# MVME-HBUT/Faster-OreFSDet

Measured on AMD Instinct MI355X. Metric: images/sec at 640x640 25-shot (eval FPS: model(inputs) + device sync per image, bs=1 per GPU), higher is better.
Workload: dtype f32

## Files before the change

### faster-orefsdet_amd/csrc/ore_conv_internal.h

```cpp
#pragma once
#include "ore_common.h"

namespace oreconv {

struct Lvl { int orow0, irow0, H, W, Ho, Wo; };

struct ConvP {
    const float* in; int in_ld, in_coff;
    int B, Cin;
    int nlev; Lvl lv[4];
    const float* w;
    int Cout, Cout16, kh, kw, stride, pad, M, K;
    const float* scale; const float* shift; int ep_stride; int relu_cout;
    const float* in_mul; const float* in_add; int in_relu;
    const float* add; int add_ld, add_coff, add_H, add_W;
    float* out; int out_ld, out_coff;
    float* colsum;
    int splitk, steps_per_split, nchunks;
    float* ws; int* tile_cnt;
    int bf16;
    int xmap;
    int sb;
    const float* wino;
    size_t w_lstride;
// ... 1 lines not shown
};

__device__ __forceinline__ void tile_of_block(int xmap, int& bx, int& by) {
    bx = blockIdx.x; by = blockIdx.y;
    if (xmap == 0) return;
    const int gx = gridDim.x, gy = gridDim.y, T = gx * gy;
    const int lin = by * gx + bx, r = lin & 7, k = lin >> 3;
    const int q = T >> 3, rem = T & 7;
    const int t = r * q + min(r, rem) + k;
    if (xmap == 1) { bx = t / gy; by = t - bx * gy; }
    else { by = t / gx; bx = t - by * gx; }
}

__device__ __forceinline__ void decode_row(const ConvP& p, int m, int& lvl, int& b, int& oy, int& ox) {
    lvl = 0;
#pragma unroll
    for (int l = 1; l < 4; ++l)
        if (l < p.nlev && m >= p.lv[l].orow0) lvl = l;
    const Lvl& L = p.lv[lvl];
    const int r = m - L.orow0, hw = L.Ho * L.Wo;
    b = r / hw;
    const int q = r - b * hw;
    oy = q / L.Wo;
    ox = q - oy * L.Wo;
}

constexpr unsigned kOOB = 0x80000000u;
constexpr int kGdTab = 64;
constexpr int kKdTab = 512;
constexpr int kRfTab = 256;

#define ORE_IGEMM_BUILDS(X)                                                                                                         \
                                                                         \
    X(128, 16, 4, 1, 1, 0) X(128, 32, 4, 1, 1, 0) X(128, 48, 4, 1, 1, 0) X(128, 64, 4, 1, 1, 0)                                     \
    X(128, 80, 4, 1, 1, 0) X(128, 96, 4, 1, 1, 0) X(128, 112, 4, 1, 1, 0) X(128, 128, 2, 2, 1, 0)                                   \
    X(64, 16, 4, 1, 1, 1) X(64, 32, 4, 1, 1, 1) X(64, 48, 4, 1, 1, 1) X(64, 64, 4, 1, 1, 1)                                         \
    X(64, 80, 4, 1, 1, 1) X(64, 96, 4, 1, 1, 1) X(64, 112, 4, 1, 1, 1) X(64, 128, 2, 2, 1, 1)                                       \
                                                                            \
    X(64, 64, 2, 1, 2, 0) X(64, 32, 2, 1, 2, 0) X(64, 16, 2, 1, 2, 0) X(64, 48, 2, 1, 2, 0)                                         \
    X(32, 64, 1, 1, 4, 0) X(32, 48, 1, 1, 4, 0) X(32, 32, 1, 1, 4, 1) X(32, 16, 1, 1, 4, 0)                                         \
    X(16, 64, 1, 1, 4, 0) X(16, 48, 1, 1, 4, 0) X(16, 32, 1, 1, 4, 1) X(16, 16, 1, 1, 4, 1)                                         \
    X(64, 128, 2, 1, 2, 0) X(64, 96, 2, 1, 2, 0) X(64, 80, 2, 1, 2, 0) X(64, 112, 2, 1, 2, 0)                                       \
    X(32, 128, 1, 1, 4, 0) X(32, 96, 1, 1, 4, 0) X(32, 80, 1, 1, 4, 0) X(32, 112, 1, 1, 4, 0)                                       \
    X(32, 128, 2, 1, 2, 0) X(32, 64, 2, 1, 2, 1) X(32, 32, 2, 1, 2, 0)                                                              \
    X(128, 64, 2, 1, 2, 0) X(128, 128, 2, 1, 2, 0)
#define ORE_GD_BUILDS(X)                                                                                                            \
    X(64, 128, 2, 2, 4, 1) X(64, 64, 2, 2, 4, 1) X(32, 64, 1, 4, 4, 1)                                                              \
    X(64, 128, 2, 2, 4, 0) X(64, 64, 2, 2, 4, 0) X(64, 112, 4, 1, 4, 0) X(128, 64, 4, 1, 4, 0) X(128, 128, 2, 2, 4, 0)              \
    X(32, 128, 1, 4, 4, 0) X(128, 112, 4, 1, 4, 0) X(208, 64, 1, 4, 4, 0) X(224, 64, 1, 4, 4, 0) X(112, 64, 1, 4, 4, 0)             \
    X(96, 128, 2, 2, 4, 0) X(64, 128, 2, 2, 2, 0) X(128, 128, 2, 2, 2, 0) X(208, 64, 1, 4, 2, 0) X(128, 112, 4, 1, 2, 0)            \
    X(128, 128, 2, 4, 4, 0) X(112, 128, 1, 8, 4, 0) X(128, 112, 8, 1, 4, 0) X(64, 128, 2, 4, 4, 0) X(128, 64, 4, 2, 4, 0)           \
    X(64, 64, 2, 4, 4, 0) X(128, 128, 2, 4, 2, 0) X(112, 128, 1, 8, 2, 0) X(80, 64, 1, 4, 4, 0) X(80, 128, 1, 4, 4, 0)              \
    X(48, 64, 1, 4, 4, 0) X(32, 64, 1, 4, 4, 0)
#define ORE_KD_BUILDS(X)                                                                                                            \
    X(16, 16, 4, 4) X(16, 16, 4, 8) X(16, 16, 8, 4) X(16, 16, 16, 2) X(16, 32, 4, 4) X(16, 32, 8, 2) X(32, 32, 4, 4) X(32, 32, 8, 2)  \
    X(16, 48, 4, 4) X(16, 48, 8, 2) X(16, 64, 4, 2) X(16, 80, 4, 2) X(32, 64, 4, 2) X(32, 80, 4, 2) X(64, 64, 4, 2) X(32, 48, 4, 2)    \
    X(32, 16, 4, 4)
#define ORE_RF_BUILDS(X) \
    X(1, 4, 8) X(1, 4, 12) X(1, 4, 16) X(1, 8, 12) X(1, 8, 16) X(1, 8, 20) X(1, 16, 12) X(2, 4, 12) X(2, 4, 16) X(2, 8, 12)
#define ORE_GS_BUILDS(X) \
    X(64, 112, 4, 1) X(64, 128, 2, 2) X(64, 64, 2, 2) X(128, 64, 4, 1) X(128, 128, 2, 2) X(32, 128, 1, 4) X(128, 112, 4, 1) X(64, 80, 4, 1) X(32, 64, 2, 2)
#define ORE_KW_TILES(X) \
    X(16, 16) X(16, 32) X(16, 48) X(16, 64) X(16, 80) X(32, 16) X(32, 32) X(32, 48) X(32, 64) X(32, 80)
constexpr bool gs_fits(int bm, int bn, int ns) { return ((bm + bn) / 16 + 3) / 4 * (ns - 1) <= 63 && (size_t)ns * (bm + bn) * 64 <= 150 * 1024; }

struct ConvKnobs {
    int patch_mode = -1;
    int kw_mode = 1;
    int kw_force[4] = {};
    int gs_force[2] = {};
    int gs_ns = 3;
    int xmap_force = -1;
    int kw_nw_force = 0;
    int wino_mode = 1;
    int ws_sb_mode = 1;
    int ws_s2_mode = 1;
    int rf_mode = 1;
    int rf_force[3] = {};
    int kd_mode = 1;
    int kd_force[4] = {};
    int gd_mode = 1;
    int gd_force[3] = {};
    int gd_dbg = 0;
    int igemm[5] = {};
};
extern ConvKnobs g_knobs;

using ConvPlan = ore_conv_plan_t;
ConvPlan conv_plan(const ConvP& p, int req_splitk, size_t workspace_floats);
bool conv_wino_covers(int Cout, int Cin);
int wino_level_blocks(const ConvP& p, int gy, int* blk0);

int launch_ws(const ConvP& p, const ConvPlan& pl, hipStream_t st);
int launch_patch(const ConvP& p, const ConvPlan& pl, hipStream_t st);
int launch_igemm(const ConvP& p, const ConvPlan& pl, hipStream_t st);
int launch_wino(const ConvP& p, const ConvPlan& pl, hipStream_t st);
int launch_gd(const ConvP& p, const ConvPlan& pl, hipStream_t st);
int launch_kd(const ConvP& p, const ConvPlan& pl, hipStream_t st);
int launch_rf(const ConvP& p, const ConvPlan& pl, hipStream_t st);
int launch_gs(const ConvP& p, const ConvPlan& pl, hipStream_t st);
int launch_kw(const ConvP& p, const ConvPlan& pl, hipStream_t st);
int conv_gd_splitk(const float* in, int in_ld, const float* w, int M, int K, int Cout16, float* parts, int S, hipStream_t st);

int launch_wgrad_reduce(const float* slab, int S, int Cout, int taps, int Cin, float beta, float* dw_oihw, long long stride, float* db,
                        float beta_b, hipStream_t st);

}
```

### faster-orefsdet_amd/csrc/ore_conv_plan.cpp

```cpp
#include "ore_common.h"
#include "ore_conv_internal.h"

namespace oreconv {

ConvKnobs g_knobs;

namespace {

const ConvKnobs& K = g_knobs;

ConvPlan make_plan(int launcher, int bm, int bn, int b0, int b1, int b2, int b3, int gx, int gy, int xmap = 0, int splitk = 1, int sps = 0) {
    ConvPlan pl{};
    pl.launcher = launcher; pl.error = ORE_OK;
    pl.bm = bm; pl.bn = bn;
    pl.build[0] = b0; pl.build[1] = b1; pl.build[2] = b2; pl.build[3] = b3;
    pl.splitk = splitk; pl.steps_per_split = sps; pl.xmap = xmap;
    pl.gx = gx; pl.gy = gy;
    return pl;
}

ConvPlan none() { return ConvPlan{}; }

ConvPlan fail(int code) {
    ConvPlan pl{};
// ... 430 lines not shown
}

}

bool conv_wino_covers(int Cout, int Cin) {
    if (Cout <= 0 || Cout % 16 != 0) return false;
    if (Cin == 64) return Cout % 64 == 0;
    if (Cin == 128) return Cout % 32 == 0;
    return Cin == 80 || Cin == 96 || Cin == 112;
}

int wino_level_blocks(const ConvP& c, int gy, int* blk0) {
    int nb[4];
    for (int l = 0; l < c.nlev; ++l) nb[l] = c.B * ceil_div(c.lv[l].W, 16) * ceil_div(c.lv[l].H, 4);
    const int G = 256 / gy > c.nlev ? 256 / gy : c.nlev;
    int R = 1;
    for (;; ++R) {
        int need = 0;
        for (int l = 0; l < c.nlev; ++l) need += ceil_div(nb[l], R);
        if (need <= G) break;
    }
    int gx = 0;
    for (int l = 0; l < c.nlev; ++l) { if (blk0) blk0[l] = gx; gx += ceil_div(nb[l], R); }
    if (blk0) blk0[c.nlev] = gx;
    return gx;
}

ConvPlan conv_plan(const ConvP& p, int req_splitk, size_t workspace_floats) {
    ConvPlan pl;
    if (p.w_lstride) {
        if ((pl = plan_ws_sb(p)).launcher) return pl;
        ore_set_error("ore_conv2d_levels_fwd: the weight-stationary bf16 kernel does not cover this per-level launch (64 / 128 channels, Cout %% 64 == 0)");
        return fail(ORE_EINVAL);
    }
    if (p.wino_lstride) {
        if ((pl = plan_wino(p)).launcher) return pl;
        ore_set_error("ore_conv2d_levels_fwd: the Winograd kernel does not cover this per-level launch (alignment / mode)");
        return fail(ORE_EINVAL);
    }
    if (p.sb & 1) {
        if ((pl = plan_ws_sb(p)).launcher || (pl = plan_ws_s2(p)).launcher) return pl;
        pl = plan_dma(p, workspace_floats);
        if (pl.launcher || pl.error) return pl;
        ore_set_error("ore_conv2d_fwd: no bf16-storage kernel for this layer (input affine?)");
        return fail(ORE_EINVAL);
    }
    if (K.igemm[0] == 0 && req_splitk <= 1) {
        if ((pl = plan_wino(p)).launcher) return pl;
        if (K.kw_mode && ((pl = plan_gd(p)).launcher || pl.error)) return pl;
        const bool kw_first = K.kw_mode == 2 || (K.kw_mode == 1 && p.nlev > 1);
        if (!kw_first && (pl = plan_patch(p)).launcher) return pl;
        if (K.kw_mode) {
            pl = plan_dma(p, workspace_floats);
            if (pl.launcher || pl.error) return pl;
            if (kw_first && K.kw_mode != 2 && (pl = plan_patch(p)).launcher) return pl;
        }
    }
    return plan_igemm(p, req_splitk, workspace_floats);
}

}

using namespace oreconv;

extern "C" int ore_conv_set_plan_override(int32_t BM, int32_t BN, int32_t WGM, int32_t WGN, int32_t WGK) {
    ConvKnobs& k = g_knobs;
    switch (BM) {
    case -1: k.patch_mode = BN; k.igemm[0] = 0; break;
    case -2: k.kw_mode = BN; k.igemm[0] = 0; break;
    case -3: k.kw_force[0] = BN; k.kw_force[1] = WGM; k.kw_force[2] = WGN; k.kw_force[3] = WGK; break;
    case -4: k.gs_force[0] = BN; k.gs_force[1] = WGM; if (WGN > 0) k.gs_ns = WGN; break;
    case -5: k.xmap_force = BN; break;
    case -6: k.kw_nw_force = BN; break;
    case -7: k.wino_mode = BN; break;
    case -8: k.ws_sb_mode = BN; break;
    case -9: k.ws_s2_mode = BN; break;
    case -10: k.rf_mode = BN; break;
    case -11: k.rf_force[0] = BN; k.rf_force[1] = WGM; k.rf_force[2] = WGN; break;
    case -12: k.kd_mode = BN; break;
    case -13: k.kd_force[0] = BN; k.kd_force[1] = WGM; k.kd_force[2] = WGN; k.kd_force[3] = WGK; break;
    case -14: k.gd_mode = BN; break;
    case -15: k.gd_force[0] = BN; k.gd_force[1] = WGM; k.gd_force[2] = WGN; break;
    case -16: k.gd_dbg = BN; break;
    default: k.igemm[0] = BM; k.igemm[1] = BN; k.igemm[2] = WGM; k.igemm[3] = WGN; k.igemm[4] = WGK; break;
    }
    return ORE_OK;
}

extern "C" int ore_conv_reset_plan_overrides(void) {
    g_knobs = ConvKnobs{};
    return ORE_OK;
}
```

### faster-orefsdet_amd/csrc/ore_misc.hip

```cpp
#include "ore_common.h"
#include "ore_ese.h"
#include <stdlib.h>
#include <algorithm>

namespace {

template <typename T, int NT, typename TO = float>
__global__ __launch_bounds__(256) void k_stem1(const T* __restrict__ img, int B, int H, int W, int Ho, int Wo,
                                               float m0, float m1, float m2, float s0, float s1, float s2,
                                               const float* __restrict__ w, const float* __restrict__ scale,
                                               const float* __restrict__ shift, int Cout, TO* __restrict__ out,
                                               int out_ld, int out_coff, int groups_per_wave) {
    constexpr int MAXNT = NT;
    const int lane = threadIdx.x & 63, wave = threadIdx.x >> 6;
    const int li = lane & 15, g = lane >> 4;
    int kdy[7], kdx[7], koff[7];
    bool kv[7];
    float kmean[7], kstd[7];
#pragma unroll
    for (int j = 0; j < 7; ++j) {
        const int k = 4 * j + g;
        kv[j] = k < 27;
        const int kk = kv[j] ? k : 0;
        const int kc = kk / 9;
        kdy[j] = (kk % 9) / 3 - 1; kdx[j] = kk % 3 - 1;
        koff[j] = (kc * H + kdy[j]) * W + kdx[j];
        kmean[j] = kc == 0 ? m0 : (kc == 1 ? m1 : m2);
        kstd[j] = kc == 0 ? s0 : (kc == 1 ? s1 : s2);
    }
    const int M = B * Ho * Wo, HoWo = Ho * Wo;
    const float inv_hw = 1.0f / (float)HoWo, inv_wo = 1.0f / (float)Wo;
    const int ngroups = (M + 15) >> 4;
    const int gw0 = (blockIdx.x * 4 + wave) * groups_per_wave;
    const bool big = M >= (1 << 22);
    auto fdiv = [](int n, int d, float inv) {
        int q = (int)((float)n * inv);
        int r = n - q * d;
        q += r >= d ? 1 : 0;
        r -= r >= d ? d : 0;
        q -= r < 0 ? 1 : 0;
        return q;
    };
    T raw[7];
    unsigned okm = 0u;
    auto gather = [&](int grp) {
        okm = 0u;
        const int pix = grp * 16 + li;
        if (grp >= ngroups || pix >= M) {
#pragma unroll
            for (int j = 0; j < 7; ++j) raw[j] = (T)0;
            return;
        }
        const int b = big ? pix / HoWo : fdiv(pix, HoWo, inv_hw), r = pix - b * HoWo;
        const int oy = fdiv(r, Wo, inv_wo), ox = r - oy * Wo;
        const int base = (b * 3 * H + oy * 2) * W + ox * 2;
#pragma unroll
        for (int j = 0; j < 7; ++j) {
            const int iy = oy * 2 + kdy[j], ix = ox * 2 + kdx[j];
            const bool ok = kv[j] && (unsigned)iy < (unsigned)H && (unsigned)ix < (unsigned)W;
            raw[j] = ok ? img[base + koff[j]] : (T)0;
            okm |= ok ? 1u << j : 0u;
        }
    };
    gather(gw0);
    __shared__ float sw[NT * 16 * 28];
    for (int i = threadIdx.x; i < NT * 16 * 28; i += 256) {
        const int n = i / 28, k = i - n * 28;
        sw[i] = k < 27 ? w[n * 27 + k] : 0.f;
    }
    f32x4 esc[MAXNT], esh[MAXNT];
#pragma unroll
    for (int t = 0; t < MAXNT; ++t) {
        esc[t] = *reinterpret_cast<const f32x4*>(scale + t * 16 + g * 4);
        esh[t] = *reinterpret_cast<const f32x4*>(shift + t * 16 + g * 4);
    }
    __syncthreads();
    float bw[MAXNT][7];
#pragma unroll
    for (int t = 0; t < MAXNT; ++t)
#pragma unroll
        for (int j = 0; j < 7; ++j) bw[t][j] = sw[(t * 16 + li) * 28 + 4 * j + g];
    for (int gi = 0; gi < groups_per_wave; ++gi) {
        const int grp = gw0 + gi;
        if (grp >= ngroups) break;
        float a[7];
#pragma unroll
        for (int j = 0; j < 7; ++j) a[j] = ((okm >> j) & 1u) ? ((float)raw[j] - kmean[j]) / kstd[j] : 0.f;
        if (gi + 1 < groups_per_wave) gather(grp + 1);
        f32x4 acc[MAXNT];
#pragma unroll
        for (int t = 0; t < MAXNT; ++t) acc[t] = f32x4{0.f, 0.f, 0.f, 0.f};
#pragma unroll
        for (int j = 0; j < 7; ++j)
#pragma unroll
            for (int t = 0; t < MAXNT; ++t)
                if (t < NT) acc[t] = __builtin_amdgcn_mfma_f32_16x16x4f32(bw[t][j], a[j], acc[t], 0, 0, 0);
        const int m = grp * 16 + li;
        if (m < M) {
            TO* orow = out + (size_t)m * out_ld + out_coff + g * 4;
#pragma unroll
            for (int t = 0; t < MAXNT; ++t) {
                if (t < NT) {
                    f32x4 v = acc[t] * esc[t] + esh[t];
                    v.x = fmaxf(v.x, 0.f); v.y = fmaxf(v.y, 0.f); v.z = fmaxf(v.z, 0.f); v.w = fmaxf(v.w, 0.f);
                    st4(orow + t * 16, v);
                }
            }
        }
    }
}

template <typename TS>
__global__ __launch_bounds__(256) void k_maxpool(const TS* __restrict__ in, int in_ld, int in_coff, int B, int H,
                                                 int W, int C4, int Ho, int Wo, const float* __restrict__ mul, int C,
                                                 TS* __restrict__ out, int out_ld, int out_coff) {
    const int idx = blockIdx.x * 256 + threadIdx.x;
    const int total = B * Ho * Wo * C4;
    if (idx >= total) return;
    const int c4 = idx % C4, pix = idx / C4;
    const int b = pix / (Ho * Wo), r = pix - b * Ho * Wo;
    const int oy = r / Wo, ox = r - oy * Wo;
    f32x4 m = {-INFINITY, -INFINITY, -INFINITY, -INFINITY};
#pragma unroll
    for (int ky = 0; ky < 3; ++ky)
#pragma unroll
        for (int kx = 0; kx < 3; ++kx) {
            const int iy = oy * 2 + ky, ix = ox * 2 + kx;
            if (iy < H && ix < W) {
                const f32x4 v = ld4(in + (size_t)((b * H + iy) * W + ix) * in_ld + in_coff + c4 * 4);
                m.x = fmaxf(m.x, v.x); m.y = fmaxf(m.y, v.y); m.z = fmaxf(m.z, v.z); m.w = fmaxf(m.w, v.w);
            }
        }
    if (mul) m = m * *reinterpret_cast<const f32x4*>(mul + b * C + c4 * 4);
    st4(out + (size_t)pix * out_ld + out_coff + c4 * 4, m);
}

template <typename TS>
__global__ __launch_bounds__(256) void k_colsum_partial(const TS* __restrict__ x, int ld, int coff, int HW, int C,
                                                        float* __restrict__ part) {
    __shared__ float red[256 * 4];
    const int b = blockIdx.y, p = blockIdx.x, P = gridDim.x;
    const int C4 = C >> 2;
    const int cpb = C4 < 256 ? C4 : 256;
    const int rpar = 256 / cpb;
    const int c4t = threadIdx.x % cpb, rr = threadIdx.x / cpb;
    const int rows_per = (HW + P - 1) / P;
    const int r0 = p * rows_per, r1 = min(r0 + rows_per, HW);
    for (int c4 = c4t; c4 < C4; c4 += cpb) {
        f32x4 acc = {0.f, 0.f, 0.f, 0.f};
        if (rr < rpar)
            for (int r = r0 + rr; r < r1; r += rpar)
                acc += ld4(x + (size_t)(b * HW + r) * ld + coff + c4 * 4);
        *reinterpret_cast<f32x4*>(red + threadIdx.x * 4) = acc;
        __syncthreads();
        if (rr == 0) {
            for (int k = 1; k < rpar; ++k) acc += *reinterpret_cast<const f32x4*>(red + (threadIdx.x + k * cpb) * 4);
            *reinterpret_cast<f32x4*>(part + ((size_t)(b * P + p)) * C + c4 * 4) = acc;
        }
        __syncthreads();
    }
}

__device__ __forceinline__ void ese_scale_columns(const EseSm& sm, int C, const float* __restrict__ lw, float* __restrict__ lws, int lrows,
                                                  int lws_bf16) {
    const int o0 = blockIdx.x * 16;
    for (int it = threadIdx.x; it < lrows * 4; it += ESE_T) {
        const int n = it >> 2, j = it & 3;
        if (o0 + j * 4 >= C) continue;
        const f32x4 w = *reinterpret_cast<const f32x4*>(lw + (size_t)n * C + o0 + j * 4);
        const f32x4 ws4 = f32x4{w.x * sm.g16[j * 4], w.y * sm.g16[j * 4 + 1], w.z * sm.g16[j * 4 + 2], w.w * sm.g16[j * 4 + 3]};
        if (lws_bf16) st4(reinterpret_cast<ore_bf16_t*>(lws) + (size_t)n * C + o0 + j * 4, ws4);
        else *reinterpret_cast<f32x4*>(lws + (size_t)n * C + o0 + j * 4) = ws4;
    }
}

__global__ __launch_bounds__(ESE_T) void k_ese_gate_fused(const float* __restrict__ part, int P, int HW, int C, const float* __restrict__ fw,
                                                          const float* __restrict__ fb, float* __restrict__ gate,
                                                          const float* __restrict__ lw, float* __restrict__ lws, int lrows, int lws_bf16) {
    __shared__ EseSm sm;
    ese_gate16(sm, part, P, HW, C, fw, fb, gate, blockIdx.y, true);
    if (lws) ese_scale_columns(sm, C, lw, lws, lrows, lws_bf16);
}

template <typename TS>
__global__ __launch_bounds__(ESE_T) void k_ese_gate_pool(const float* __restrict__ part, int P, int HW, int C, const float* __restrict__ fw,
                                                         const float* __restrict__ fb, float* __restrict__ gate,
                                                         const float* __restrict__ lw, float* __restrict__ lws, int lrows, int lws_bf16,
                                                         const TS* __restrict__ in, int in_ld, int in_coff, int H, int W, int Ho, int Wo,
                                                         TS* __restrict__ out, int out_ld, int out_coff) {
    __shared__ EseSm sm;
// ... 296 lines not shown
    __syncthreads();
    if (threadIdx.x < G) {
        float t = 0.f;
        for (int k = 0; k < rpar; ++k) t += red[k * G + threadIdx.x];
        float* o = stats + ((size_t)blockIdx.x * G + threadIdx.x) * 2;
        o[0] = gmean[threadIdx.x]; o[1] = t;
    }
}

struct GnCombineSm { float sn[8][64], sm[8][64], sq[8][64], fmean[64], frstd[64]; };
__device__ __forceinline__ void gn_combine_block(GnCombineSm& S, const float* __restrict__ stats, const GnSeg& sg, int b, int C, int G, float eps,
                                                 const float* __restrict__ gamma, const float* __restrict__ beta, float* omul, float* oadd) {
    const int lvl = b / sg.B, img = b - lvl * sg.B;
    const int nchunks = sg.nchunk[lvl], HW = sg.HW[lvl];
    stats += (size_t)(sg.chunk0[lvl] + img * nchunks) * G * 2;
    const int cpg = C / G;
    const int gdiv = G > 32 ? 64 : 32, nsl = 256 / gdiv;
    const int g = threadIdx.x % gdiv, sl = threadIdx.x / gdiv;
    float n = 0.f, mean = 0.f, m2 = 0.f;
    if (g < G)
        for (int c0 = sl; c0 < nchunks; c0 += nsl * 8) {
            float2 rec[8];
#pragma unroll
            for (int k = 0; k < 8; ++k) {
                const int ch = c0 + nsl * k;
                rec[k] = ch < nchunks ? *reinterpret_cast<const float2*>(stats + ((size_t)ch * G + g) * 2) : float2{0.f, 0.f};
            }
#pragma unroll
            for (int k = 0; k < 8; ++k) {
                const int ch = c0 + nsl * k;
                if (ch < nchunks) {
                    const float nb = (float)((min((ch + 1) * GN_ROWS, HW) - ch * GN_ROWS) * cpg);
                    const float mb = rec[k].x, qb = rec[k].y;
                    const float nt = n + nb, d = mb - mean;
                    mean += d * (nb / nt);
                    m2 += qb + d * d * (n * nb / nt);
                    n = nt;
                }
            }
        }
    S.sn[sl][g] = n; S.sm[sl][g] = mean; S.sq[sl][g] = m2;
    __syncthreads();
    if (threadIdx.x < G) {
        float N = S.sn[0][g], M = S.sm[0][g], Q = S.sq[0][g];
        for (int k = 1; k < nsl; ++k) {
            const float nb = S.sn[k][g];
            if (nb > 0.f) {
                const float nt = N + nb, d = S.sm[k][g] - M;
                M += d * (nb / nt);
                Q += S.sq[k][g] + d * d * (N * nb / nt);
                N = nt;
            }
        }
        S.fmean[g] = M;
        S.frstd[g] = 1.0f / sqrtf(Q / N + eps);
    }
    __syncthreads();
    for (int c = threadIdx.x; c < C; c += 256) {
        const float m = S.frstd[c / cpg] * gamma[c];
        omul[c] = m;
        oadd[c] = beta[c] - S.fmean[c / cpg] * m;
    }
}

__global__ __launch_bounds__(256) void k_gn_combine(const float* __restrict__ stats, GnSeg sg, int C, int G, float eps,
                                                    const float* __restrict__ gamma, const float* __restrict__ beta,
                                                    float* __restrict__ mul, float* __restrict__ add) {
    __shared__ GnCombineSm S;
    const int b = blockIdx.x;
    gn_combine_block(S, stats, sg, b, C, G, eps, gamma, beta, mul + (size_t)b * C, add + (size_t)b * C);
}


struct HeadP {
    const void* tow; int ld;
    int B, nlev; int H[4], W[4], row0[4], tile0[5], tx[4], ty[4];
    const float* mul; const float* add;
    const float* w;
    const float* scale; const float* shift; int ep_stride;
    float* out; int out_ld;
    const float* stats; GnSeg sg; const float* gamma; const float* beta; float eps; int G;
};

template <typename TS>
__global__ __launch_bounds__(256) void k_head_pred(HeadP p) {
    constexpr int C = 128, Q = 32, NO = 5, TP = 8, HP = TP + 2;
    __shared__ __attribute__((aligned(16))) float sX[HP * HP * C];
    __shared__ __attribute__((aligned(16))) float sW[NO * 9 * C];
    const int tid = threadIdx.x;
    int lvl = 0;
#pragma unroll
    for (int l = 1; l < 4; ++l)
        if (l < p.nlev && (int)blockIdx.x >= p.tile0[l]) lvl = l;
    const int H = p.H[lvl], W = p.W[lvl];
    const int tl = blockIdx.x - p.tile0[lvl], per = p.tx[lvl] * p.ty[lvl];
    const int b = tl / per, tr = tl - b * per;
    const int y0 = (tr / p.tx[lvl]) * TP, x0 = (tr % p.tx[lvl]) * TP;
    const int base = p.row0[lvl] + b * H * W;
    const TS* tow = reinterpret_cast<const TS*>(p.tow);
    __shared__ __attribute__((aligned(16))) float s_mul[C], s_add[C];
    __shared__ GnCombineSm S;
    constexpr int NX = (HP * HP * Q + 255) / 256;
    constexpr int NWV = (NO * 9 * Q + 255) / 256;
    f32x4 xv[NX], wv[NWV];
#pragma unroll
    for (int k = 0; k < NWV; ++k) {
        const int i = tid + k * 256;
        wv[k] = i < NO * 9 * Q ? *reinterpret_cast<const f32x4*>(p.w + i * 4) : f32x4{0.f, 0.f, 0.f, 0.f};
    }
#pragma unroll
    for (int k = 0; k < NX; ++k) {
        const int i = tid + k * 256;
        const int px = i / Q, q = i - px * Q;
        const int gy = y0 - 1 + px / HP, gx = x0 - 1 + px % HP;
        const bool ok = i < HP * HP * Q && (unsigned)gy < (unsigned)H && (unsigned)gx < (unsigned)W;
        xv[k] = ok ? ld4(tow + (size_t)(base + gy * W + gx) * p.ld + q * 4) : f32x4{0.f, 0.f, 0.f, 0.f};
    }
    if (p.stats) gn_combine_block(S, p.stats, p.sg, lvl * p.B + b, C, p.G, p.eps, p.gamma, p.beta, s_mul, s_add);
    else if (tid < C) { s_mul[tid] = p.mul[(size_t)(lvl * p.B + b) * C + tid]; s_add[tid] = p.add[(size_t)(lvl * p.B + b) * C + tid]; }
    __syncthreads();
    const float* mul = s_mul;
    const float* add = s_add;
#pragma unroll
    for (int k = 0; k < NWV; ++k) {
        const int i = tid + k * 256;
        if (i < NO * 9 * Q) *reinterpret_cast<f32x4*>(sW + i * 4) = wv[k];
    }
#pragma unroll
    for (int k = 0; k < NX; ++k) {
        const int i = tid + k * 256;
        if (i < HP * HP * Q) {
            const int px = i / Q, q = i - px * Q;
            const int gy = y0 - 1 + px / HP, gx = x0 - 1 + px % HP;
            f32x4 v = {0.f, 0.f, 0.f, 0.f};
            if ((unsigned)gy < (unsigned)H && (unsigned)gx < (unsigned)W) {
                v = xv[k] * *reinterpret_cast<const f32x4*>(mul + q * 4) + *reinterpret_cast<const f32x4*>(add + q * 4);
                v.x = fmaxf(v.x, 0.f); v.y = fmaxf(v.y, 0.f); v.z = fmaxf(v.z, 0.f); v.w = fmaxf(v.w, 0.f);
            }
            *reinterpret_cast<f32x4*>(sX + i * 4) = v;
        }
    }
    __syncthreads();
    const int q = tid & 31, r = tid >> 5;
    float acc[TP][NO];
#pragma unroll
    for (int x = 0; x < TP; ++x)
#pragma unroll
        for (int o = 0; o < NO; ++o) acc[x][o] = 0.f;
#pragma unroll
    for (int dy = 0; dy < 3; ++dy) {
        f32x4 xr[HP];
#pragma unroll
        for (int x = 0; x < HP; ++x) xr[x] = *reinterpret_cast<const f32x4*>(sX + (((r + dy) * HP + x) * Q + q) * 4);
#pragma unroll
        for (int dx = 0; dx < 3; ++dx)
#pragma unroll
            for (int o = 0; o < NO; ++o) {
                const f32x4 w4 = *reinterpret_cast<const f32x4*>(sW + ((o * 9 + dy * 3 + dx) * Q + q) * 4);
#pragma unroll
                for (int x = 0; x < TP; ++x) {
                    const f32x4 v = xr[x + dx];
                    acc[x][o] = fmaf(v.x, w4.x, fmaf(v.y, w4.y, fmaf(v.z, w4.z, fmaf(v.w, w4.w, acc[x][o]))));
                }
            }
    }
    __syncthreads();
    float* part = sX;
#pragma unroll
    for (int x = 0; x < TP; ++x)
#pragma unroll
        for (int o = 0; o < NO; ++o) part[((r * TP + x) * NO + o) * Q + q] = acc[x][o];
    __syncthreads();
    for (int i = tid; i < TP * TP * NO; i += 256) {
        const int px = i / NO, o = i - px * NO;
        const float* pp = part + i * Q;
        float s0 = 0.f, s1 = 0.f, s2 = 0.f, s3 = 0.f;
#pragma unroll
        for (int k = 0; k < Q; k += 4) { s0 += pp[k]; s1 += pp[k + 1]; s2 += pp[k + 2]; s3 += pp[k + 3]; }
        float v = (s0 + s1) + (s2 + s3);
        const int gy = y0 + px / TP, gx = x0 + px % TP;
        if (gy < H && gx < W) {
            v = v * p.scale[lvl * p.ep_stride + o] + p.shift[lvl * p.ep_stride + o];
            if (o < 4) v = fmaxf(v, 0.f);
            p.out[(size_t)(base + gy * W + gx) * p.out_ld + o] = v;
        }
    }
}

}

struct HeadGn { const float* stats; GnSeg sg; const float* gamma; const float* beta; float eps; int G; };
static int head_pred_launch(const void* tower, int32_t ld, int32_t B, int32_t n_levels, const int32_t* H, const int32_t* W, const float* mul,
                            const float* add, const float* w_packed16, const float* scale, const float* shift, int32_t ep_stride,
                            float* out, int32_t out_ld, void* stream, int bf16, const HeadGn* gn = nullptr) {
    ORE_CHECK_ARG(tower && H && W && (gn || (mul && add)) && w_packed16 && scale && shift && out, "ore_head_pred_fwd: null pointer");
    ORE_CHECK_ARG(B > 0 && n_levels >= 1 && n_levels <= 4 && ld >= 128 && ld % 4 == 0 && out_ld >= 5, "ore_head_pred_fwd: bad args");
    HeadP p{};
    p.tow = tower; p.ld = ld; p.B = B; p.nlev = n_levels;
    int rows = 0, tiles = 0;
    for (int l = 0; l < n_levels; ++l) {
        ORE_CHECK_ARG(H[l] > 0 && W[l] > 0, "ore_head_pred_fwd: level %d geometry", l);
        p.H[l] = H[l]; p.W[l] = W[l]; p.row0[l] = rows; p.tile0[l] = tiles;
        p.tx[l] = ceil_div(W[l], 8); p.ty[l] = ceil_div(H[l], 8);
        rows += B * H[l] * W[l]; tiles += B * p.tx[l] * p.ty[l];
    }
    p.tile0[n_levels] = tiles;
    p.mul = mul; p.add = add; p.w = w_packed16; p.scale = scale; p.shift = shift; p.ep_stride = ep_stride; p.out = out; p.out_ld = out_ld;
    if (gn) { p.stats = gn->stats; p.sg = gn->sg; p.gamma = gn->gamma; p.beta = gn->beta; p.eps = gn->eps; p.G = gn->G; }
    if (bf16) hipLaunchKernelGGL(k_head_pred<ore_bf16_t>, dim3(tiles), dim3(256), 0, (hipStream_t)stream, p);
    else hipLaunchKernelGGL(k_head_pred<float>, dim3(tiles), dim3(256), 0, (hipStream_t)stream, p);
    return ore_launch_status("k_head_pred");
}

extern "C" int ore_head_pred_fwd(const float* tower, int32_t ld, int32_t B, int32_t n_levels, const int32_t* H, const int32_t* W,
                                 const float* gn_mul, const float* gn_add, const float* w_packed16, const float* scale, const float* shift,
                                 int32_t ep_stride, float* out, int32_t out_ld, void* stream) {
    return head_pred_launch(tower, ld, B, n_levels, H, W, gn_mul, gn_add, w_packed16, scale, shift, ep_stride, out, out_ld, stream, 0);
}

extern "C" int ore_head_pred_bf16_fwd(const uint16_t* tower, int32_t ld, int32_t B, int32_t n_levels, const int32_t* H, const int32_t* W,
                                      const float* gn_mul, const float* gn_add, const float* w_packed16, const float* scale,
                                      const float* shift, int32_t ep_stride, float* out, int32_t out_ld, void* stream) {
    return head_pred_launch(tower, ld, B, n_levels, H, W, gn_mul, gn_add, w_packed16, scale, shift, ep_stride, out, out_ld, stream, 1);
}

static int stem1_launch(const void* img, int32_t img_is_u8, int32_t B, int32_t H, int32_t W, int32_t Hp,
                             int32_t Wp, const float* mean3, const float* std3, const float* w_oihw,
                             const float* scale, const float* shift, int32_t Cout, void* out, int32_t out_ld,
                             int32_t out_coff, void* stream, int out_bf16) {
    ORE_CHECK_ARG(img && mean3 && std3 && w_oihw && scale && shift && out, "ore_stem1_fwd: null pointer");
    ORE_CHECK_ARG(B > 0 && H > 0 && W > 0 && Hp >= H && Wp >= W && Hp % 2 == 0 && Wp % 2 == 0, "ore_stem1_fwd: geometry");
    ORE_CHECK_ARG(Cout % 16 == 0 && Cout <= 128 && out_coff % 4 == 0 && out_ld % 4 == 0 && out_coff + Cout <= out_ld,
                  "ore_stem1_fwd: Cout=%d ld=%d coff=%d", Cout, out_ld, out_coff);
    const int Ho = Hp / 2, Wo = Wp / 2;
    const int M = B * Ho * Wo;
    ore_flop_count_add(2.0 * (double)M * Cout * 27.0);
    ORE_CHECK_ARG((long long)Ho * Wo < (1ll << 22) && (long long)B * Ho * Wo < (1ll << 31) && (long long)B * 3 * H * W < (1ll << 31),
                  "ore_stem1_fwd: %d images of %dx%d exceed the kernel's 32-bit indexing", B, H, W);
    hipStream_t st = (hipStream_t)stream;
    const int ngroups = ceil_div(M, 16);
    const int gpw = ngroups >= 2048 ? 2 : 1;
    const int blocks = ceil_div(ngroups, 4 * gpw);
#define ORE_STEM1(T, NT)                                                                                              \
    do { if (out_bf16) hipLaunchKernelGGL((k_stem1<T, NT, ore_bf16_t>), dim3(blocks), dim3(256), 0, st, (const T*)img, B, H, W, Ho, Wo, mean3[0], mean3[1], \
                       mean3[2], std3[0], std3[1], std3[2], w_oihw, scale, shift, Cout, (ore_bf16_t*)out, out_ld, out_coff, gpw); \
    else hipLaunchKernelGGL((k_stem1<T, NT, float>), dim3(blocks), dim3(256), 0, st, (const T*)img, B, H, W, Ho, Wo, mean3[0], mean3[1], \
                       mean3[2], std3[0], std3[1], std3[2], w_oihw, scale, shift, Cout, (float*)out, out_ld, out_coff, gpw); } while (0)
    switch ((Cout >> 4) * 2 + (img_is_u8 ? 1 : 0)) {
        case 2: ORE_STEM1(float, 1); break;     case 3: ORE_STEM1(uint8_t, 1); break;
        case 4: ORE_STEM1(float, 2); break;     case 5: ORE_STEM1(uint8_t, 2); break;
        case 8: ORE_STEM1(float, 4); break;     case 9: ORE_STEM1(uint8_t, 4); break;
        case 16: ORE_STEM1(float, 8); break;    case 17: ORE_STEM1(uint8_t, 8); break;
        default: ore_set_error("ore_stem1_fwd: Cout=%d not in {16,32,64,128}", Cout); return ORE_EINVAL;
    }
#undef ORE_STEM1
    return ore_launch_status("k_stem1");
}

extern "C" int ore_stem1_fwd(const void* img, int32_t img_is_u8, int32_t B, int32_t H, int32_t W, int32_t Hp,
                             int32_t Wp, const float* mean3, const float* std3, const float* w_oihw,
                             const float* scale, const float* shift, int32_t Cout, float* out, int32_t out_ld,
                             int32_t out_coff, void* stream) {
    return stem1_launch(img, img_is_u8, B, H, W, Hp, Wp, mean3, std3, w_oihw, scale, shift, Cout, out, out_ld, out_coff, stream, 0);
}

extern "C" int ore_stem1_bf16_fwd(const void* img, int32_t img_is_u8, int32_t B, int32_t H, int32_t W, int32_t Hp,
                                  int32_t Wp, const float* mean3, const float* std3, const float* w_oihw,
                                  const float* scale, const float* shift, int32_t Cout, uint16_t* out, int32_t out_ld,
                                  int32_t out_coff, void* stream) {
    return stem1_launch(img, img_is_u8, B, H, W, Hp, Wp, mean3, std3, w_oihw, scale, shift, Cout, out, out_ld, out_coff, stream, 1);
}

extern "C" int ore_maxpool3x3s2_fwd(const float* in, int32_t in_ld, int32_t in_coff, int32_t B, int32_t H, int32_t W,
                                    int32_t C, const float* in_mul, float* out, int32_t out_ld, int32_t out_coff,
                                    void* stream) {
    ORE_CHECK_ARG(in && out && B > 0 && H >= 1 && W >= 1 && C % 4 == 0, "ore_maxpool3x3s2_fwd: bad args");
    ORE_CHECK_ARG(in_ld % 4 == 0 && in_coff % 4 == 0 && out_ld % 4 == 0 && out_coff % 4 == 0, "ore_maxpool3x3s2_fwd: align");
    auto osz = [](int n) { int o = (n - 3 + 1) / 2 + 1; if (n < 3) o = 1; if ((o - 1) * 2 >= n) --o; return o < 1 ? 1 : o; };
    const int Ho = osz(H), Wo = osz(W);
    const int total = B * Ho * Wo * (C / 4);
    hipLaunchKernelGGL(k_maxpool<float>, dim3(ceil_div(total, 256)), dim3(256), 0, (hipStream_t)stream, in, in_ld, in_coff, B, H,
                       W, C / 4, Ho, Wo, in_mul, C, out, out_ld, out_coff);
    return ore_launch_status("k_maxpool");
}

extern "C" int ore_maxpool3x3s2_bf16_fwd(const uint16_t* in, int32_t in_ld, int32_t in_coff, int32_t B, int32_t H, int32_t W,
                                         int32_t C, const float* in_mul, uint16_t* out, int32_t out_ld, int32_t out_coff, void* stream) {
    ORE_CHECK_ARG(in && out && B > 0 && H >= 1 && W >= 1 && C % 4 == 0, "ore_maxpool3x3s2_bf16_fwd: bad args");
    ORE_CHECK_ARG(in_ld % 4 == 0 && in_coff % 4 == 0 && out_ld % 4 == 0 && out_coff % 4 == 0, "ore_maxpool3x3s2_bf16_fwd: align");
    auto osz = [](int n) { int o = (n - 3 + 1) / 2 + 1; if (n < 3) o = 1; if ((o - 1) * 2 >= n) --o; return o < 1 ? 1 : o; };
    const int Ho = osz(H), Wo = osz(W);
    const int total = B * Ho * Wo * (C / 4);
    hipLaunchKernelGGL(k_maxpool<ore_bf16_t>, dim3(ceil_div(total, 256)), dim3(256), 0, (hipStream_t)stream, (const ore_bf16_t*)in, in_ld,
                       in_coff, B, H, W, C / 4, Ho, Wo, in_mul, C, (ore_bf16_t*)out, out_ld, out_coff);
    return ore_launch_status("k_maxpool");
}

extern "C" int ore_ese_gate_fwd(const float* x, int32_t ld, int32_t coff, int32_t B, int32_t HW, int32_t C,
                                const float* fc_w, const float* fc_b, float* gate, float* workspace, void* stream) {
    ORE_CHECK_ARG(x && fc_w && fc_b && gate && workspace, "ore_ese_gate_fwd: null pointer");
    ORE_CHECK_ARG(B > 0 && HW > 0 && C % 4 == 0 && C <= 4096 && ld % 4 == 0 && coff % 4 == 0, "ore_ese_gate_fwd: bad args");
    hipStream_t st = (hipStream_t)stream;
    int P = ceil_div(HW, 32);
    if (P > ORE_ESE_PARTS) P = ORE_ESE_PARTS;
    hipLaunchKernelGGL(k_colsum_partial<float>, dim3(P, B), dim3(256), 0, st, x, ld, coff, HW, C, workspace);
    int rc = ore_launch_status("k_colsum_partial");
    if (rc) return rc;
    hipLaunchKernelGGL(k_ese_gate_fused, dim3(ceil_div(C, 16), B), dim3(ESE_T), 0, st, workspace, P, HW, C, fc_w, fc_b, gate,
                       (const float*)nullptr, (float*)nullptr, 0, 0);
    return ore_launch_status("k_ese_gate_fused");
}

extern "C" int ore_ese_gate_bf16_fwd(const uint16_t* x, int32_t ld, int32_t coff, int32_t B, int32_t HW, int32_t C,
                                     const float* fc_w, const float* fc_b, float* gate, float* workspace, void* stream) {
    ORE_CHECK_ARG(x && fc_w && fc_b && gate && workspace, "ore_ese_gate_bf16_fwd: null pointer");
    ORE_CHECK_ARG(B > 0 && HW > 0 && C % 4 == 0 && C <= 4096 && ld % 4 == 0 && coff % 4 == 0, "ore_ese_gate_bf16_fwd: bad args");
    hipStream_t st = (hipStream_t)stream;
    int P = ceil_div(HW, 32);
    if (P > ORE_ESE_PARTS) P = ORE_ESE_PARTS;
    hipLaunchKernelGGL(k_colsum_partial<ore_bf16_t>, dim3(P, B), dim3(256), 0, st, reinterpret_cast<const ore_bf16_t*>(x), ld, coff, HW, C,
                       workspace);
    int rc = ore_launch_status("k_colsum_partial");
    if (rc) return rc;
    hipLaunchKernelGGL(k_ese_gate_fused, dim3(ceil_div(C, 16), B), dim3(ESE_T), 0, st, workspace, P, HW, C, fc_w, fc_b, gate,
                       (const float*)nullptr, (float*)nullptr, 0, 0);
    return ore_launch_status("k_ese_gate_fused");
}

extern "C" int ore_ese_gate_from_colsum_fwd(const float* part, int32_t P, int32_t B, int32_t HW, int32_t C, const float* fc_w,
                                            const float* fc_b, float* gate, float* mean_ws, void* stream) {
    ORE_CHECK_ARG(part && fc_w && fc_b && gate && mean_ws && P > 0 && B > 0 && HW > 0 && C > 0 && C % 4 == 0 && C <= 4096,
                  "ore_ese_gate_from_colsum_fwd: bad args");
    hipStream_t st = (hipStream_t)stream;
    hipLaunchKernelGGL(k_ese_gate_fused, dim3(ceil_div(C, 16), B), dim3(ESE_T), 0, st, part, P, HW, C, fc_w, fc_b, gate,
                       (const float*)nullptr, (float*)nullptr, 0, 0);
    return ore_launch_status("k_ese_gate_fused");
}

// ... 237 lines not shown
```

### faster-orefsdet_amd/csrc/ore_util.cpp

```cpp
#include <stdarg.h>
#include <stdio.h>
#include "ore_hip.h"

static thread_local char g_err[512] = "";

void ore_set_error(const char* fmt, ...) {
    va_list ap;
    va_start(ap, fmt);
    vsnprintf(g_err, sizeof(g_err), fmt, ap);
    va_end(ap);
}

extern "C" const char* ore_last_error(void) { return g_err; }

#include <atomic>
static std::atomic<double> g_flops{0.0};
static std::atomic<long long> g_flop_calls{0};
void ore_flop_count_add(double flops) {
    double cur = g_flops.load(std::memory_order_relaxed);
    while (!g_flops.compare_exchange_weak(cur, cur + flops, std::memory_order_relaxed)) {}
    g_flop_calls.fetch_add(1, std::memory_order_relaxed);
}
static thread_local int g_last_wino = 0;
void ore_note_wino(int v) { g_last_wino = v; }
int ore_last_wino(void) { return g_last_wino; }
static thread_local int g_last_launch = ORE_LAUNCH_NONE, g_last_split = 1;
void ore_note_launch(int code, int split) { g_last_launch = code; g_last_split = split; }
extern "C" int32_t ore_conv_last_launch(int32_t* split) {
    if (split) *split = g_last_split;
    return g_last_launch;
}
extern "C" int ore_flop_counter_read(double* flops, int64_t* calls, int32_t reset) {
    if (flops) *flops = g_flops.load(std::memory_order_relaxed);
    if (calls) *calls = (int64_t)g_flop_calls.load(std::memory_order_relaxed);
    if (reset) { g_flops.store(0.0, std::memory_order_relaxed); g_flop_calls.store(0, std::memory_order_relaxed); }
    return ORE_OK;
}
extern "C" double ore_dwpw_flops(int64_t rows, int32_t C) { return 2.0 * (double)rows * (double)C * (9.0 + (double)C); }
extern "C" int32_t ore_det_record_rows(void) { return ORE_DET_RECORD_ROWS; }
extern "C" int ore_version(void) { return 601; }
```

Baseline: 1707.

## Use grid-stride persistent stem kernel and shorter head-pred tiles

The stem conv kernel now launches at most as many blocks as can be resident, sized by an occupancy query, and each wave walks groups with a grid stride while prefetching the next group. The head prediction kernel now uses 8x4 spatial tiles instead of 8x8, doubling block count and splitting each warp's x range. Both changes are meant to improve GPU fill and load balance for small bs=1 feature maps. A knob restores the old forms. Costs are an extra one-time occupancy query, more halo reloads per tile in the head kernel, and a partial-tile reduction.

```diff
diff --git a/faster-orefsdet_amd/csrc/ore_conv_internal.h b/faster-orefsdet_amd/csrc/ore_conv_internal.h
--- a/faster-orefsdet_amd/csrc/ore_conv_internal.h
+++ b/faster-orefsdet_amd/csrc/ore_conv_internal.h
@@ -107,6 +107,7 @@
     int gd_mode = 1;
     int gd_force[3] = {};
     int gd_dbg = 0;
+    int floor_prev = 0;
     int igemm[5] = {};
 };
 extern ConvKnobs g_knobs;
diff --git a/faster-orefsdet_amd/csrc/ore_conv_plan.cpp b/faster-orefsdet_amd/csrc/ore_conv_plan.cpp
--- a/faster-orefsdet_amd/csrc/ore_conv_plan.cpp
+++ b/faster-orefsdet_amd/csrc/ore_conv_plan.cpp
@@ -536,6 +536,7 @@
     case -14: k.gd_mode = BN; break;
     case -15: k.gd_force[0] = BN; k.gd_force[1] = WGM; k.gd_force[2] = WGN; break;
     case -16: k.gd_dbg = BN; break;
+    case -17: k.floor_prev = BN; break;
     default: k.igemm[0] = BM; k.igemm[1] = BN; k.igemm[2] = WGM; k.igemm[3] = WGN; k.igemm[4] = WGK; break;
     }
     return ORE_OK;
diff --git a/faster-orefsdet_amd/csrc/ore_misc.hip b/faster-orefsdet_amd/csrc/ore_misc.hip
--- a/faster-orefsdet_amd/csrc/ore_misc.hip
+++ b/faster-orefsdet_amd/csrc/ore_misc.hip
@@ -1,11 +1,12 @@
 #include "ore_common.h"
+#include "ore_conv_internal.h"
 #include "ore_ese.h"
 #include <stdlib.h>
 #include <algorithm>
 
 namespace {
 
-template <typename T, int NT, typename TO = float>
+template <typename T, int NT, typename TO = float, int FORM = 1>
 __global__ __launch_bounds__(256) void k_stem1(const T* __restrict__ img, int B, int H, int W, int Ho, int Wo,
                                                float m0, float m1, float m2, float s0, float s1, float s2,
                                                const float* __restrict__ w, const float* __restrict__ scale,
@@ -31,7 +32,8 @@
     const int M = B * Ho * Wo, HoWo = Ho * Wo;
     const float inv_hw = 1.0f / (float)HoWo, inv_wo = 1.0f / (float)Wo;
     const int ngroups = (M + 15) >> 4;
-    const int gw0 = (blockIdx.x * 4 + wave) * groups_per_wave;
+    const int nw = (int)gridDim.x * 4;
+    const int gw0 = (blockIdx.x * 4 + wave) * (FORM != 0 ? 1 : groups_per_wave);
     const bool big = M >= (1 << 22);
     auto fdiv = [](int n, int d, float inv) {
         int q = (int)((float)n * inv);
@@ -80,13 +82,7 @@
     for (int t = 0; t < MAXNT; ++t)
 #pragma unroll
         for (int j = 0; j < 7; ++j) bw[t][j] = sw[(t * 16 + li) * 28 + 4 * j + g];
-    for (int gi = 0; gi < groups_per_wave; ++gi) {
-        const int grp = gw0 + gi;
-        if (grp >= ngroups) break;
-        float a[7];
-#pragma unroll
-        for (int j = 0; j < 7; ++j) a[j] = ((okm >> j) & 1u) ? ((float)raw[j] - kmean[j]) / kstd[j] : 0.f;
-        if (gi + 1 < groups_per_wave) gather(grp + 1);
+    auto mul_store = [&](int grp, const float (&a)[7]) {
         f32x4 acc[MAXNT];
 #pragma unroll
         for (int t = 0; t < MAXNT; ++t) acc[t] = f32x4{0.f, 0.f, 0.f, 0.f};
@@ -106,6 +102,25 @@
                     st4(orow + t * 16, v);
                 }
             }
+        }
+    };
+    if constexpr (FORM == 1) {
+        for (int grp = gw0; grp < ngroups; grp += nw) {
+            float a[7];
+#pragma unroll
+            for (int j = 0; j < 7; ++j) a[j] = ((okm >> j) & 1u) ? ((float)raw[j] - kmean[j]) / kstd[j] : 0.f;
+            if (grp + nw < ngroups) gather(grp + nw);
+            mul_store(grp, a);
+        }
+    } else {
+        for (int gi = 0; gi < groups_per_wave; ++gi) {
+            const int grp = gw0 + gi;
+            if (grp >= ngroups) break;
+            float a[7];
+#pragma unroll
+            for (int j = 0; j < 7; ++j) a[j] = ((okm >> j) & 1u) ? ((float)raw[j] - kmean[j]) / kstd[j] : 0.f;
+            if (gi + 1 < groups_per_wave) gather(grp + 1);
+            mul_store(grp, a);
         }
     }
 }
@@ -568,10 +583,10 @@
     const float* stats; GnSeg sg; const float* gamma; const float* beta; float eps; int G;
 };
 
-template <typename TS>
+template <typename TS, int TPY>
 __global__ __launch_bounds__(256) void k_head_pred(HeadP p) {
-    constexpr int C = 128, Q = 32, NO = 5, TP = 8, HP = TP + 2;
-    __shared__ __attribute__((aligned(16))) float sX[HP * HP * C];
+    constexpr int C = 128, Q = 32, NO = 5, TP = 8, HP = TP + 2, HPY = TPY + 2, XT = TP * TPY / 8, XH = XT + 2;
+    __shared__ __attribute__((aligned(16))) float sX[HPY * HP * C];
     __shared__ __attribute__((aligned(16))) float sW[NO * 9 * C];
     const int tid = threadIdx.x;
     int lvl = 0;
@@ -581,12 +596,12 @@
     const int H = p.H[lvl], W = p.W[lvl];
     const int tl = blockIdx.x - p.tile0[lvl], per = p.tx[lvl] * p.ty[lvl];
     const int b = tl / per, tr = tl - b * per;
-    const int y0 = (tr / p.tx[lvl]) * TP, x0 = (tr % p.tx[lvl]) * TP;
+    const int y0 = (tr / p.tx[lvl]) * TPY, x0 = (tr % p.tx[lvl]) * TP;
     const int base = p.row0[lvl] + b * H * W;
     const TS* tow = reinterpret_cast<const TS*>(p.tow);
     __shared__ __attribute__((aligned(16))) float s_mul[C], s_add[C];
     __shared__ GnCombineSm S;
-    constexpr int NX = (HP * HP * Q + 255) / 256;
+    constexpr int NX = (HPY * HP * Q + 255) / 256;
     constexpr int NWV = (NO * 9 * Q + 255) / 256;
     f32x4 xv[NX], wv[NWV];
 #pragma unroll
@@ -599,7 +614,7 @@
         const int i = tid + k * 256;
         const int px = i / Q, q = i - px * Q;
         const int gy = y0 - 1 + px / HP, gx = x0 - 1 + px % HP;
-        const bool ok = i < HP * HP * Q && (unsigned)gy < (unsigned)H && (unsigned)gx < (unsigned)W;
+        const bool ok = i < HPY * HP * Q && (unsigned)gy < (unsigned)H && (unsigned)gx < (unsigned)W;
         xv[k] = ok ? ld4(tow + (size_t)(base + gy * W + gx) * p.ld + q * 4) : f32x4{0.f, 0.f, 0.f, 0.f};
     }
     if (p.stats) gn_combine_block(S, p.stats, p.sg, lvl * p.B + b, C, p.G, p.eps, p.gamma, p.beta, s_mul, s_add);
@@ -615,7 +630,7 @@
 #pragma unroll
     for (int k = 0; k < NX; ++k) {
         const int i = tid + k * 256;
-        if (i < HP * HP * Q) {
+        if (i < HPY * HP * Q) {
             const int px = i / Q, q = i - px * Q;
             const int gy = y0 - 1 + px / HP, gx = x0 - 1 + px % HP;
             f32x4 v = {0.f, 0.f, 0.f, 0.f};
@@ -627,24 +642,25 @@
         }
     }
     __syncthreads();
-    const int q = tid & 31, r = tid >> 5;
-    float acc[TP][NO];
-#pragma unroll
-    for (int x = 0; x < TP; ++x)
+    const int q = tid & 31;
+    const int r = (tid >> 5) * XT / TP, xb = ((tid >> 5) * XT) % TP;
+    float acc[XT][NO];
+#pragma unroll
+    for (int x = 0; x < XT; ++x)
 #pragma unroll
         for (int o = 0; o < NO; ++o) acc[x][o] = 0.f;
 #pragma unroll
     for (int dy = 0; dy < 3; ++dy) {
-        f32x4 xr[HP];
-#pragma unroll
-        for (int x = 0; x < HP; ++x) xr[x] = *reinterpret_cast<const f32x4*>(sX + (((r + dy) * HP + x) * Q + q) * 4);
+        f32x4 xr[XH];
+#pragma unroll
+        for (int x = 0; x < XH; ++x) xr[x] = *reinterpret_cast<const f32x4*>(sX + (((r + dy) * HP + xb + x) * Q + q) * 4);
 #pragma unroll
         for (int dx = 0; dx < 3; ++dx)
 #pragma unroll
             for (int o = 0; o < NO; ++o) {
                 const f32x4 w4 = *reinterpret_cast<const f32x4*>(sW + ((o * 9 + dy * 3 + dx) * Q + q) * 4);
 #pragma unroll
-                for (int x = 0; x < TP; ++x) {
+                for (int x = 0; x < XT; ++x) {
                     const f32x4 v = xr[x + dx];
                     acc[x][o] = fmaf(v.x, w4.x, fmaf(v.y, w4.y, fmaf(v.z, w4.z, fmaf(v.w, w4.w, acc[x][o]))));
                 }
@@ -653,11 +669,11 @@
     __syncthreads();
     float* part = sX;
 #pragma unroll
-    for (int x = 0; x < TP; ++x)
-#pragma unroll
-        for (int o = 0; o < NO; ++o) part[((r * TP + x) * NO + o) * Q + q] = acc[x][o];
-    __syncthreads();
-    for (int i = tid; i < TP * TP * NO; i += 256) {
+    for (int x = 0; x < XT; ++x)
+#pragma unroll
+        for (int o = 0; o < NO; ++o) part[((r * TP + xb + x) * NO + o) * Q + q] = acc[x][o];
+    __syncthreads();
+    for (int i = tid; i < TPY * TP * NO; i += 256) {
         const int px = i / NO, o = i - px * NO;
         const float* pp = part + i * Q;
         float s0 = 0.f, s1 = 0.f, s2 = 0.f, s3 = 0.f;
@@ -683,18 +699,24 @@
     ORE_CHECK_ARG(B > 0 && n_levels >= 1 && n_levels <= 4 && ld >= 128 && ld % 4 == 0 && out_ld >= 5, "ore_head_pred_fwd: bad args");
     HeadP p{};
     p.tow = tower; p.ld = ld; p.B = B; p.nlev = n_levels;
+    const int tpy = (oreconv::g_knobs.floor_prev & 2) ? 8 : 4;
     int rows = 0, tiles = 0;
     for (int l = 0; l < n_levels; ++l) {
         ORE_CHECK_ARG(H[l] > 0 && W[l] > 0, "ore_head_pred_fwd: level %d geometry", l);
         p.H[l] = H[l]; p.W[l] = W[l]; p.row0[l] = rows; p.tile0[l] = tiles;
-        p.tx[l] = ceil_div(W[l], 8); p.ty[l] = ceil_div(H[l], 8);
+        p.tx[l] = ceil_div(W[l], 8); p.ty[l] = ceil_div(H[l], tpy);
         rows += B * H[l] * W[l]; tiles += B * p.tx[l] * p.ty[l];
     }
     p.tile0[n_levels] = tiles;
     p.mul = mul; p.add = add; p.w = w_packed16; p.scale = scale; p.shift = shift; p.ep_stride = ep_stride; p.out = out; p.out_ld = out_ld;
     if (gn) { p.stats = gn->stats; p.sg = gn->sg; p.gamma = gn->gamma; p.beta = gn->beta; p.eps = gn->eps; p.G = gn->G; }
-    if (bf16) hipLaunchKernelGGL(k_head_pred<ore_bf16_t>, dim3(tiles), dim3(256), 0, (hipStream_t)stream, p);
-    else hipLaunchKernelGGL(k_head_pred<float>, dim3(tiles), dim3(256), 0, (hipStream_t)stream, p);
+    if (tpy == 8) {
+        if (bf16) hipLaunchKernelGGL((k_head_pred<ore_bf16_t, 8>), dim3(tiles), dim3(256), 0, (hipStream_t)stream, p);
+        else hipLaunchKernelGGL((k_head_pred<float, 8>), dim3(tiles), dim3(256), 0, (hipStream_t)stream, p);
+    } else {
+        if (bf16) hipLaunchKernelGGL((k_head_pred<ore_bf16_t, 4>), dim3(tiles), dim3(256), 0, (hipStream_t)stream, p);
+        else hipLaunchKernelGGL((k_head_pred<float, 4>), dim3(tiles), dim3(256), 0, (hipStream_t)stream, p);
+    }
     return ore_launch_status("k_head_pred");
 }
 
@@ -708,6 +730,16 @@
                                       const float* gn_mul, const float* gn_add, const float* w_packed16, const float* scale,
                                       const float* shift, int32_t ep_stride, float* out, int32_t out_ld, void* stream) {
     return head_pred_launch(tower, ld, B, n_levels, H, W, gn_mul, gn_add, w_packed16, scale, shift, ep_stride, out, out_ld, stream, 1);
+}
+
+static int resident_blocks(const void* kernel) {
+    int dev = 0, cus = 0, per_cu = 0;
+    if (hipGetDevice(&dev) != hipSuccess || hipDeviceGetAttribute(&cus, hipDeviceAttributeMultiprocessorCount, dev) != hipSuccess ||
+        hipOccupancyMaxActiveBlocksPerMultiprocessor(&per_cu, kernel, 256, 0) != hipSuccess || cus < 1 || per_cu < 1) {
+        ore_set_error("k_stem1: occupancy query failed (%d compute units, %d blocks each)", cus, per_cu);
+        return 0;
+    }
+    return cus * per_cu;
 }
 
 static int stem1_launch(const void* img, int32_t img_is_u8, int32_t B, int32_t H, int32_t W, int32_t Hp,
@@ -727,11 +759,16 @@
     const int ngroups = ceil_div(M, 16);
     const int gpw = ngroups >= 2048 ? 2 : 1;
     const int blocks = ceil_div(ngroups, 4 * gpw);
-#define ORE_STEM1(T, NT)                                                                                              \
-    do { if (out_bf16) hipLaunchKernelGGL((k_stem1<T, NT, ore_bf16_t>), dim3(blocks), dim3(256), 0, st, (const T*)img, B, H, W, Ho, Wo, mean3[0], mean3[1], \
-                       mean3[2], std3[0], std3[1], std3[2], w_oihw, scale, shift, Cout, (ore_bf16_t*)out, out_ld, out_coff, gpw); \
-    else hipLaunchKernelGGL((k_stem1<T, NT, float>), dim3(blocks), dim3(256), 0, st, (const T*)img, B, H, W, Ho, Wo, mean3[0], mean3[1], \
-                       mean3[2], std3[0], std3[1], std3[2], w_oihw, scale, shift, Cout, (float*)out, out_ld, out_coff, gpw); } while (0)
+    const bool prev = (oreconv::g_knobs.floor_prev & 1) != 0;
+    int rc1 = ORE_OK;
+#define ORE_STEM1_K(T, NT, TO)                                                                                        \
+    do { if (prev) hipLaunchKernelGGL((k_stem1<T, NT, TO, 0>), dim3(blocks), dim3(256), 0, st, (const T*)img, B, H, W, Ho, Wo, mean3[0], mean3[1], \
+                       mean3[2], std3[0], std3[1], std3[2], w_oihw, scale, shift, Cout, (TO*)out, out_ld, out_coff, gpw); \
+    else { static const int slots = resident_blocks((const void*)k_stem1<T, NT, TO, 1>);                              \
+           if (slots < 1) { rc1 = ORE_EHIP; break; }                                                                  \
+           hipLaunchKernelGGL((k_stem1<T, NT, TO, 1>), dim3(std::min(ceil_div(ngroups, 4), slots)), dim3(256), 0, st, (const T*)img, B, H, W, Ho, Wo, mean3[0], mean3[1], \
+                       mean3[2], std3[0], std3[1], std3[2], w_oihw, scale, shift, Cout, (TO*)out, out_ld, out_coff, gpw); } } while (0)
+#define ORE_STEM1(T, NT) do { if (out_bf16) ORE_STEM1_K(T, NT, ore_bf16_t); else ORE_STEM1_K(T, NT, float); } while (0)
     switch ((Cout >> 4) * 2 + (img_is_u8 ? 1 : 0)) {
         case 2: ORE_STEM1(float, 1); break;     case 3: ORE_STEM1(uint8_t, 1); break;
         case 4: ORE_STEM1(float, 2); break;     case 5: ORE_STEM1(uint8_t, 2); break;
@@ -740,6 +777,8 @@
         default: ore_set_error("ore_stem1_fwd: Cout=%d not in {16,32,64,128}", Cout); return ORE_EINVAL;
     }
 #undef ORE_STEM1
+#undef ORE_STEM1_K
+    if (rc1) return rc1;
     return ore_launch_status("k_stem1");
 }
 
diff --git a/faster-orefsdet_amd/csrc/ore_util.cpp b/faster-orefsdet_amd/csrc/ore_util.cpp
--- a/faster-orefsdet_amd/csrc/ore_util.cpp
+++ b/faster-orefsdet_amd/csrc/ore_util.cpp
@@ -38,4 +38,4 @@
 }
 extern "C" double ore_dwpw_flops(int64_t rows, int32_t C) { return 2.0 * (double)rows * (double)C * (9.0 + (double)C); }
 extern "C" int32_t ore_det_record_rows(void) { return ORE_DET_RECORD_ROWS; }
-extern "C" int ore_version(void) { return 601; }
+extern "C" int ore_version(void) { return 700; }
```

Measured after the change: 1706. About the same (-0.1%).
